# Kyubyong/dc_tts

Hardware: NVIDIA H100
Metric: mel_frames_per_sec (higher is better)
Workload: dtype f32 (decode: fp32 FMA; TextEnc/SSRN: fp16x2 split operands on wgmma, fp32 accumulate)

## Files before the change

### dc_tts_b200/csrc/dctts_api.cu

```cuda
#include "../../include/dctts.h"
#include "kernels.cuh"
#include "kernels_tc.cuh"
#include "kernels_decode.cuh"

#include <cstdio>
#include <cstdlib>
#include <algorithm>
#include <cmath>
#include <cstring>
#include <map>
#include <memory>
#include <stdexcept>
#include <string>
#include <vector>

using namespace dctts;

#define CUDA_CHECK(expr)                                                                     \
    do {                                                                                     \
        cudaError_t _e = (expr);                                                             \
        if (_e != cudaSuccess) {                                                             \
            char _buf[512];                                                                  \
            snprintf(_buf, sizeof(_buf), "%s failed: %s (%s:%d)", #expr, cudaGetErrorString(_e), \
                     __FILE__, __LINE__);                                                    \
// ... 370 lines not shown
    memset(&P, 0, sizeof(P));
    P.nl = (int)nets.size(); P.n_enc = (int)h->audioenc.size();
    std::vector<int> prow = audiodec_rows(h->audiodec, hp.max_T);
    int nch = 0, off = 0;
    for (int li = 0; li < P.nl; ++li) {
        const LayerDev& l = *nets[li];
        DecLayer& L = P.L[li];
        if (l.kind == K_D || !l.causal || (l.cin % 4) || (l.kind == K_HC && (l.cin != d || l.cout != d)) || l.cout % DEC_NC ||
            (li != 0 && l.cin % 128)) { D.why = "persistent decode: unsupported block " + l.scope; return; }
        L.kind = l.kind == K_HC ? 1 : 0; L.cin = l.cin; L.cout = l.cout; L.ntaps = l.size; L.rate = l.rate; L.act = l.act;
        L.cs = l.cout / DEC_NC; L.ns = L.kind ? 2 * L.cs : (L.cs <= 8 ? 8 : roundup(L.cs, 4));
        if (L.ns != 8 && L.ns != 16 && L.ns != 32) { D.why = "persistent decode: unsupported slice width"; return; }
        L.prow = li >= P.n_enc ? prow[li - P.n_enc] : 1;
        if (L.prow > 1 && (L.cout != 256 || (L.ns != 32 && L.ns != 16) || L.prow > 85)) { D.why = "persistent decode: unsupported receptive field"; return; }
        L.ldin = l.cin;
        const int cinp = roundup(l.cin, 128);
        if (l.size > 1 && cinp != 256) { D.why = "persistent decode: multi-tap blocks must have 256 input channels"; return; }
        const int K = l.size * cinp;
        L.krows = std::min(K, DEC_SLOT_F / L.ns);
        const int kr8 = L.krows / 8, sg = 32 / L.ns;
        if (K % L.krows || L.krows % 8 || kr8 * L.ns > DEC_REG_F || kr8 % (8 * sg) || (L.prow > 1 && kr8 % 16)) {
            D.why = "persistent decode: chunk geometry"; return;
        }
        if (L.prow > 1 && (L.prow - 1) + (l.size - 1) * l.rate > 96) { D.why = "persistent decode: receptive field too tall"; return; }
        L.ch0 = nch;
        for (int k0 = 0; k0 < K; k0 += L.krows) {
            if (nch >= DEC_MAXCH) { D.why = "persistent decode: too many weight chunks"; return; }
            DecChunk& c = P.C[nch++];
            c.off = off; c.nfl4 = (short)(L.krows * L.ns / 4); c.k0 = (short)k0; c.krows = (short)L.krows; c.layer = (short)li;
            off += L.krows * L.ns;
        }
        L.nch = nch - L.ch0;
        if (li == P.n_enc - 1) P.nch_enc = nch;
        if (L.prow > 1) { if (P.pyr_ch1 == 0) P.pyr_ch0 = L.ch0; P.pyr_ch1 = nch; }
    }
    if (P.L[P.nl - 1].prow != 1 || P.L[P.n_enc].ntaps != 1 || P.nch_enc <= DEC_NSLOT) { D.why = "persistent decode: unexpected AudioDec shape"; return; }
    for (int li = P.n_enc; li < P.nl; ++li)
        if (P.L[li].prow > 1 && li > P.n_enc && P.L[li - 1].prow <= 1) { D.why = "persistent decode: receptive-field blocks not contiguous"; return; }
    P.nch = nch;
    for (int li = 0; li < P.nl; ++li) {
        const DecLayer& L = P.L[li];
        if (L.prow <= 1) continue;
        if (L.krows % 128 || !((L.ns == 32 && L.ntaps == 3) || (L.ns == 16 && L.ntaps == 1)) ||
            (li == P.n_enc && (L.cin != 2 * d || d != 256)) || (li > P.n_enc && L.cin != 256)) {
            D.why = "persistent decode: tensor-core pre-pass geometry"; return;
        }
        for (int c = L.ch0; c < L.ch0 + L.nch; ++c) { P.C[c].off16 = off; off += L.krows * L.ns; }
// ... 499 lines not shown
    cudaError_t e = cudaGraphInstantiate(&h->ar_exec, graph, 0);
    cudaGraphDestroy(graph);
    CUDA_CHECK(e);
    CUDA_CHECK(cudaGetLastError());
    h->ar_B = B;
}

bool decode_cluster(H* h, int B, int steps, cudaStream_t s) {
    auto& D = h->dec;
    if (!D.ok || h->opt.decode_mode != 1) return false;
    const dctts_hparams& hp = h->hp;
    IntBufs ib = ints(h);
    DecParams P = D.tab;
    for (int li = 0; li < P.nl; ++li) {
        const bool enc = li < P.n_enc;
        P.out_hist[li] = enc ? h->ae_out[li].as<float>() : h->ad_out[li - P.n_enc].as<float>();
        P.in_hist[li] = li == 0 ? nullptr : (li == P.n_enc ? h->rbuf.as<float>() : P.out_hist[li - 1]);
    }
    P.kv = h->kv.as<float>(); P.ybuf = h->ybuf.as<float>(); P.rbuf = h->rbuf.as<float>(); P.pre_scr = D.scr.as<float>();
    decode_plane_halfs(h, h->ws_B, D.pl.as<__half>(), &P);
    P.p_hist = ib.p_hist; P.p_final = D.pfinal.as<int>(); P.stats = D.stats.as<int>();
    P.prof = nullptr;
    P.force_prepass = h->opt.decode_force_prepass != 0;
    if (h->opt.decode_prof) { D.prof.ensure(16 * sizeof(long long)); CUDA_CHECK(cudaMemsetAsync(D.prof.p, 0, 16 * sizeof(long long), s)); P.prof = D.prof.as<long long>(); }
    P.B = B;
    {
        const int mc = std::max(1, D.max_clusters);
        int G = 1;
        while (G < DEC_GMAX && (B + G - 1) / G > mc) ++G;
        P.G = G;
    }
    P.T = hp.max_T; P.N = hp.max_N; P.d = hp.d; P.n_mels = hp.n_mels;
    P.win_size = hp.attention_win_size; P.steps = steps;
    const int n_clusters = (B + P.G - 1) / P.G;
    cudaError_t e = launch_decode_cluster(P, n_clusters, s);
    if (e != cudaSuccess) {
        cudaGetLastError();
        D.ok = false; D.why = std::string("decode_cluster_kernel launch failed: ") + cudaGetErrorString(e);
        return false;
    }
    h->launches += 1;
    D.last_clusters = n_clusters; D.last_moved_frames = -1;
    return true;
}

void text2mel_generate(H* h, const int* L, int B, int steps, float* Y, int* prev_hist,
                       long long* maxatt, float* align, cudaStream_t s) {
// ... 1327 lines not shown
        *value = *slot;
    });
}

int dctts_decode_stats(dctts_handle h, int32_t* moved_frames, int32_t* moved_utterance_frames, int32_t* clusters) {
    return guarded(h, [&] {
        auto& D = h->dec;
        REQUIRE(D.last_clusters > 0, "dctts_decode_stats: no persistent decode has run on this handle");
        if (D.last_moved_frames < 0) {
            std::vector<int> st(2 * (size_t)D.last_clusters);
            CUDA_CHECK(cudaDeviceSynchronize());
            CUDA_CHECK(cudaMemcpy(st.data(), D.stats.p, st.size() * sizeof(int), cudaMemcpyDeviceToHost));
            D.last_moved_frames = 0; D.last_moved_utt = 0;
            for (int c = 0; c < D.last_clusters; ++c) { D.last_moved_frames += st[2 * c]; D.last_moved_utt += st[2 * c + 1]; }
        }
        if (moved_frames) *moved_frames = D.last_moved_frames;
        if (moved_utterance_frames) *moved_utterance_frames = D.last_moved_utt;
        if (clusters) *clusters = D.last_clusters;
    });
}

int dctts_decode_profile(dctts_handle h, int64_t* cycles, int32_t n) {
    return guarded(h, [&] {
        REQUIRE(cycles && n >= 1 && n <= 16, "dctts_decode_profile: bad arguments");
        REQUIRE(h->dec.prof.p, "dctts_decode_profile: no profiled decode has run (set option decode_prof)");
        CUDA_CHECK(cudaDeviceSynchronize());
        long long v[16];
        CUDA_CHECK(cudaMemcpy(v, h->dec.prof.p, sizeof(v), cudaMemcpyDeviceToHost));
        for (int i = 0; i < n; ++i) cycles[i] = v[i];
    });
}

int dctts_malloc(dctts_handle h, void** ptr, int64_t bytes) {
    return guarded(h, [&] { REQUIRE(ptr && bytes > 0, "dctts_malloc: bad arguments"); CUDA_CHECK(cudaMalloc(ptr, (size_t)bytes)); });
}
int dctts_free(dctts_handle h, void* ptr) { return guarded(h, [&] { CUDA_CHECK(cudaFree(ptr)); }); }
int dctts_memcpy_h2d(dctts_handle h, void* dst, const void* src, int64_t bytes, void* stream) {
    return guarded(h, [&] { CUDA_CHECK(cudaMemcpyAsync(dst, src, (size_t)bytes, cudaMemcpyHostToDevice, S(h, stream))); });
}
int dctts_memcpy_d2h(dctts_handle h, void* dst, const void* src, int64_t bytes, void* stream) {
    return guarded(h, [&] { CUDA_CHECK(cudaMemcpyAsync(dst, src, (size_t)bytes, cudaMemcpyDeviceToHost, S(h, stream))); });
}
int dctts_malloc_host(dctts_handle h, void** ptr, int64_t bytes) {
    return guarded(h, [&] { REQUIRE(ptr && bytes > 0, "dctts_malloc_host: bad arguments"); CUDA_CHECK(cudaMallocHost(ptr, (size_t)bytes)); });
}
int dctts_free_host(dctts_handle h, void* ptr) { return guarded(h, [&] { CUDA_CHECK(cudaFreeHost(ptr)); }); }
int dctts_stream_sync(dctts_handle h, void* stream) { return guarded(h, [&] { CUDA_CHECK(cudaStreamSynchronize(S(h, stream))); }); }

}
```

### dc_tts_b200/csrc/kernels_decode.cu

```cuda
#include "kernels_decode.cuh"
#include "tc_ptx.cuh"

#include <cuda_fp16.h>
#include <atomic>
#include <math.h>

namespace dctts {
using namespace ptx;

namespace {

constexpr int NC = DEC_NC, GMAX = DEC_GMAX, NT = DEC_THREADS, NWARP = NT / 32;
constexpr int XLD = 768;
constexpr int PLD = GMAX * 32 + 16;
constexpr int TC_RA = 96;
constexpr int TC_APLANE = 2 * TC_RA * 16;
constexpr int TC_ASTAGE = 2 * TC_APLANE;
constexpr int TC_NSTG = 3;
static_assert(GMAX * NT >= 1024, "red: LayerNorm parameters of the pre-pass");
static_assert(TC_RA == DEC_PL_PAD, "pl_c1 rows are staged as whole slabs");

struct Smem {
    float ring[DEC_NSLOT][NWARP][DEC_REG_F];
    float red[GMAX][NT];
    float xin[2][GMAX][XLD];
    union {
        float pre[2][NC][PLD];
        unsigned char tca[TC_NSTG][TC_ASTAGE];
    };
    float outv[2][GMAX * 32];
    float prm[2][DEC_PRM_F];
    unsigned long long fullw[DEC_NSLOT][NWARP];
    unsigned long long gbar[2];
    unsigned long long sbar[TC_NSTG], abar[TC_NSTG];
    float stat[GMAX][2][2];
    uint32_t tc_baddr[96];
    int n_moved_frames, n_moved_utt;
    DecParams P;
    int p_cur[GMAX], p_prev[GMAX], p_next[GMAX], moved[GMAX];
    int fmoved[2];
    long long prof[16], prof_last;
};

static_assert(sizeof(Smem) + 128 <= 232448, "decode kernel: shared memory budget (227 KB per CTA)");
static_assert(sizeof(float) * 2 * NC * PLD >= TC_NSTG * TC_ASTAGE, "A stages inside pre");

#define LAP(i) do { if constexpr (PROF) { if (threadIdx.x == 0) { const long long now_ = clock64(); S.prof[i] += now_ - S.prof_last; S.prof_last = now_; } } } while (0)
enum { LP_START = 0, LP_WAIT = 1, LP_GEMV = 2, LP_RELEASE = 3, LP_GATHER = 4, LP_CBAR = 5, LP_LN = 6, LP_MIX = 7, LP_ATT = 8,
       LP_PYR_ATT = 9, LP_PYR_GEMM = 10, LP_PYR_LN = 11, LP_PYR_BAR = 12, LP_FRAME = 13 };

__device__ __forceinline__ float warp_sum(float v) {
#pragma unroll
    for (int o = 16; o > 0; o >>= 1) v += __shfl_xor_sync(0xffffffffu, v, o);
    return v;
}
__device__ __forceinline__ float sigmoid_acc(float x) { return 1.0f / (1.0f + expf(-x)); }
__device__ __forceinline__ float sigmoid_fast(float x) { return __fdividef(1.0f, 1.0f + __expf(-x)); }

__device__ __forceinline__ void cp_async16(void* dst, const void* src, bool valid) {
    const int sz = valid ? 16 : 0;
    asm volatile("cp.async.cg.shared.global [%0], [%1], 16, %2;" :: "r"(smem_u32(dst)), "l"(src), "r"(sz) : "memory");
}
__device__ __forceinline__ void cp_async_commit() { asm volatile("cp.async.commit_group;" ::: "memory"); }
template <int N> __device__ __forceinline__ void cp_async_wait() { asm volatile("cp.async.wait_group %0;" :: "n"(N) : "memory"); }

__device__ __forceinline__ void bulk_g2s(void* dst, const void* src, uint32_t bytes, unsigned long long* bar) {
    asm volatile("cp.async.bulk.shared::cluster.global.mbarrier::complete_tx::bytes [%0], [%1], %2, [%3];"
                 :: "r"(smem_u32(dst)), "l"(src), "r"(bytes), "r"(smem_u32(bar)) : "memory");
}
__device__ __forceinline__ void bulk_s2peer(uint32_t dst_cluster, const void* src, uint32_t bytes, uint32_t bar_cluster) {
    asm volatile("cp.async.bulk.shared::cluster.shared::cta.mbarrier::complete_tx::bytes [%0], [%1], %2, [%3];"
                 :: "r"(dst_cluster), "r"(smem_u32(src)), "r"(bytes), "r"(bar_cluster) : "memory");
}
__device__ __forceinline__ void cluster_sync_all() { cluster_arrive(); cluster_wait(); }
__device__ __forceinline__ void fence_proxy_async_global() { asm volatile("fence.proxy.async.global;" ::: "memory"); }

__device__ __forceinline__ size_t pl_idx(int nslab, int rows, int b, int c, int t) {
    return ((size_t)(b * nslab + (c >> 4)) * 4 + ((c >> 3) & 1)) * (size_t)rows * 8 + (size_t)(t + DEC_PL_PAD) * 8 + (c & 7);
}
__device__ __forceinline__ void split_h(float v, __half& hi, __half& lo) {
    hi = __float2half_rn(v);
    lo = __float2half_rn(v - __half2float(hi));
}
__device__ __forceinline__ void store_split8(__half* p, const float (&v)[8]) {
    __align__(16) __half hi[8];
    __align__(16) __half lo[8];
#pragma unroll
    for (int i = 0; i < 8; ++i) split_h(v[i], hi[i], lo[i]);
    *reinterpret_cast<uint4*>(p) = *reinterpret_cast<const uint4*>(hi);
    *reinterpret_cast<uint4*>(p + TC_APLANE / 2) = *reinterpret_cast<const uint4*>(lo);
}
// ... 339 lines not shown
    r.n = j - r.t_lo;
    r.total = r.n * __popc(r.mask);
    return r;
}
__device__ __forceinline__ void pre_row_of(const PreRows& r, int m, int& g, int& t) {
    const int k = m / r.n;
    unsigned mk = r.mask;
    for (int i = 0; i < k; ++i) mk &= mk - 1;
    g = __ffs(mk) - 1;
    t = r.t_lo + (m - k * r.n);
}
__device__ __forceinline__ int pre_off_of(const PreRows& r, int g) { return r.n * __popc(r.mask & ((1u << g) - 1u)); }

__device__ __forceinline__ void pyr_tc_table(const DecParams& P, Smem& S, int li, unsigned pos0) {
    const DecLayer& l = P.L[li];
    const int nslab = l.cin / 16, spc = l.krows / 16, spr = spc / 8, slab_f = 16 * l.ns;
    const int sid = (int)threadIdx.x;
    if (sid < l.ntaps * nslab) {
        const int c = sid / spc, wi = sid - c * spc, reg = wi / spr, jj = wi - reg * spr;
        S.tc_baddr[sid] = (smem_u32(&S.ring[(pos0 + c) % DEC_NSLOT][reg][jj * slab_f]) & 0x3FFFFu) >> 4;
    }
}

template <int NS, int NTAPS, int MH>
__device__ __forceinline__ void pyr_mma_rows(const DecParams& P, Smem& S, int li, unsigned& use, int& stg, int n_out, int rank,
                                             float* scr_rows) {
    const DecLayer& l = P.L[li];
    const int nslab = l.cin / 16, lane = threadIdx.x & 31, w4 = (threadIdx.x >> 5) & 3;
    const bool leader = (threadIdx.x & 127) == 0;
    unsigned char* As = &S.tca[0][0];
    const uint64_t dA0 = gmma_desc_noswz(0, TC_RA * 16, 128), dB0 = gmma_desc_noswz(0, (uint32_t)NS * 16, 128);
    const uint32_t a_base = (smem_u32(As) & 0x3FFFFu) >> 4, b_lo = (uint32_t)NS * 2, tap_step = (uint32_t)l.rate;
    float acc[MH][NS / 2];
#pragma unroll
    for (int m = 0; m < MH; ++m)
#pragma unroll
        for (int i = 0; i < NS / 2; ++i) acc[m][i] = 0.f;
    int prev = 0;
#pragma unroll 1
    for (int ks = 0; ks < nslab; ++ks) {
        uint32_t bt[NTAPS];
#pragma unroll
        for (int tap = 0; tap < NTAPS; ++tap) bt[tap] = S.tc_baddr[tap * nslab + ks];
        const uint32_t aa = a_base + (uint32_t)stg * (TC_ASTAGE >> 4);
        mbar_wait(bar64(&S.abar[stg]), use & 1u);
        wg_fence();
#pragma unroll
        for (int tap = 0; tap < NTAPS; ++tap) {
            const uint64_t db_hi = dB0 | bt[tap], db_lo = dB0 | (bt[tap] + b_lo);
#pragma unroll
            for (int m = 0; m < MH; ++m) {
                const uint32_t a = aa + (uint32_t)tap * tap_step + 64u * m;
                const uint64_t da_hi = dA0 | a, da_lo = dA0 | (a + (TC_APLANE >> 4));
                wgmma_f16<NS / 16>(acc[m], da_hi, db_hi, (ks | tap) != 0);
                wgmma_f16<NS / 16>(acc[m], da_hi, db_lo, 1u);
                wgmma_f16<NS / 16>(acc[m], da_lo, db_hi, 1u);
            }
        }
        wg_commit();
        wg_wait<1>();
        if (ks > 0 && leader) mbar_arrive(bar64(&S.sbar[prev]));
        prev = stg;
        if (++stg == TC_NSTG) { stg = 0; ++use; }
    }
    wg_wait<0>();
#pragma unroll
    for (int m = 0; m < MH; ++m) wg_fence_regs(acc[m]);
    if (leader) mbar_arrive(bar64(&S.sbar[prev]));
    const float inv = P.inv_scale[li];
    const float* bs = P.bias[li];
#pragma unroll
    for (int m = 0; m < MH; ++m)
#pragma unroll
        for (int h = 0; h < 2; ++h) {
            const int row = 64 * m + 16 * w4 + (lane >> 2) + 8 * h;
            if (row >= n_out) continue;
            float* orow = scr_rows + (size_t)row * 512;
#pragma unroll
            for (int i = 0; i < NS / 8; ++i) {
                const int n = i * 8 + 2 * (lane & 3), hf = n >> 4, nn = n & 15;
                const int col = hf * 256 + rank * 16 + nn, bi = hf * l.cout + rank * 16 + nn;
                const float2 bq = __ldg(reinterpret_cast<const float2*>(bs + bi));
                *reinterpret_cast<float2*>(orow + col) = make_float2(fmaf(acc[m][i * 4 + 2 * h], inv, bq.x),
                                                                     fmaf(acc[m][i * 4 + 2 * h + 1], inv, bq.y));
            }
        }
}

__device__ __forceinline__ void pyr_tc_utt(const DecParams& P, Smem& S, int li, unsigned q0, int b, int t_lo, int n_out,
                                        int rank, float* scr_rows, const __half* c1) {
    const DecLayer& l = P.L[li];
    const int tid = threadIdx.x, warp = tid >> 5;
    unsigned use = q0 / TC_NSTG;
    int stg = (int)(q0 - use * TC_NSTG);
    if (tid == 0) {
        const int halo = (l.ntaps - 1) * l.rate, n_src = n_out + halo;
        const int nslab = l.cin / 16;
        const size_t run = (size_t)P.pl_rows * 8;
        const __half* src = c1 ? c1 : P.pl_hist[li] + pl_idx(nslab, P.pl_rows, b, 0, t_lo - halo);
        const size_t sstep = c1 ? (size_t)TC_ASTAGE / 2 : 4 * run;
        const uint32_t rb = (uint32_t)n_src * 16;
        fence_proxy_async_global();
#pragma unroll 1
        for (int ks = 0; ks < nslab; ++ks, src += sstep) {
            if (use > 0) mbar_wait(bar64(&S.sbar[stg]), (use - 1) & 1u);
            unsigned char* dst = &S.tca[stg][0];
            if (c1) {
                mbar_expect_tx(bar64(&S.abar[stg]), TC_ASTAGE);
                bulk_g2s(dst, src, TC_ASTAGE, &S.abar[stg]);
            } else {
                mbar_expect_tx(bar64(&S.abar[stg]), 4 * rb);
#pragma unroll
                for (int r = 0; r < 4; ++r)
                    bulk_g2s(dst + (r >> 1) * TC_APLANE + (r & 1) * (TC_RA * 16), src + r * run, rb, &S.abar[stg]);
            }
            if (++stg == TC_NSTG) { stg = 0; ++use; }
        }
    } else if (warp >= 4) {
        if (l.ns == 32) {
            if (n_out > 64) pyr_mma_rows<32, 3, 2>(P, S, li, use, stg, n_out, rank, scr_rows);
            else pyr_mma_rows<32, 3, 1>(P, S, li, use, stg, n_out, rank, scr_rows);
        } else {
            if (n_out > 64) pyr_mma_rows<16, 1, 2>(P, S, li, use, stg, n_out, rank, scr_rows);
            else pyr_mma_rows<16, 1, 1>(P, S, li, use, stg, n_out, rank, scr_rows);
        }
    }
}

__device__ __forceinline__ void pyr_ln(const DecParams& P, Smem& S, int li, int b0, const PreRows& rl, int rank, const float* scr) {
    const DecLayer& l = P.L[li];
    const int warp = threadIdx.x >> 5, lane = threadIdx.x & 31;
    const float* prm = &S.red[0][0];
    const float fC = 256.f;
    for (int m = rank * NWARP + warp; m < rl.total; m += NC * NWARP) {
        int g, t; pre_row_of(rl, m, g, t);
        const float* y = scr + (size_t)m * 512;
        const size_t row = (size_t)(b0 + g) * P.T + t;
        float z[2][8];
#pragma unroll
        for (int hf = 0; hf < 2; ++hf) {
            if (hf > l.kind) break;
            const float4 a = ldcg4(y + hf * 256 + lane * 4), b = ldcg4(y + hf * 256 + 128 + lane * 4);
            float v[8] = {a.x, a.y, a.z, a.w, b.x, b.y, b.z, b.w};
            float s = 0.f;
#pragma unroll
            for (int i = 0; i < 8; ++i) s += v[i];
            const float mean = warp_sum(s) / fC;
            float qd = 0.f;
// ... 43 lines not shown
                float qv[8], ctx[8];
                const float4 q0 = ldcg4(Qh + row * P.d + lane * 8), q1 = ldcg4(Qh + row * P.d + lane * 8 + 4);
                qv[0] = q0.x; qv[1] = q0.y; qv[2] = q0.z; qv[3] = q0.w; qv[4] = q1.x; qv[5] = q1.y; qv[6] = q1.z; qv[7] = q1.w;
                attend_row(P, qv, b0 + g, S.p_cur[g], lane, ctx);
                float* rr = P.rbuf + row * (2 * P.d);
                *reinterpret_cast<float4*>(rr + lane * 8) = make_float4(ctx[0], ctx[1], ctx[2], ctx[3]);
                *reinterpret_cast<float4*>(rr + lane * 8 + 4) = make_float4(ctx[4], ctx[5], ctx[6], ctx[7]);
                *reinterpret_cast<float4*>(rr + P.d + lane * 8) = q0;
                *reinterpret_cast<float4*>(rr + P.d + lane * 8 + 4) = q1;
                __half* cs = c1s + (size_t)g * c1_utt + (size_t)(lane >> 1) * (TC_ASTAGE / 2) + (lane & 1) * (TC_RA * 8) + (t - ra.t_lo) * 8;
                store_split8(cs, ctx);
                store_split8(cs + (size_t)(P.d >> 4) * (TC_ASTAGE / 2), qv);
            }
            fence_proxy_async_global();
            cluster_sync_all();
            LAP(LP_PYR_ATT);
            for (int lp = P.n_enc; lp < P.nl && P.L[lp].prow > 1; ++lp) {
                const DecLayer& l = P.L[lp];
                for (int c = 0; c < l.nch; ++c) {
                    const unsigned pp = st.pos + c;
                    if (lane < NWARP) mbar_wait(bar64(&S.fullw[pp % DEC_NSLOT][lane]), (pp / DEC_NSLOT) & 1u);
                }
                __syncwarp();
                const PreRows rl = pre_rows(S, G, j, l.prow);
                if (rl.n > 0) {
                    pyr_tc_table(P, S, lp, st.pos);
                    __syncthreads();
                    for (int g = 0; g < G; ++g) {
                        if (!((rl.mask >> g) & 1u)) continue;
                        float* rows = scr + (size_t)pre_off_of(rl, g) * 512;
                        pyr_tc_utt(P, S, lp, st.tcq, b0 + g, rl.t_lo, rl.n, rank, rows, lp == P.n_enc ? c1s + (size_t)g * c1_utt : nullptr);
                        st.tcq += l.cin / 16;
                    }
                }
                __syncthreads();
                for (int c = 0; c < l.nch; ++c) {
                    if (lane == 0) { fence_proxy_async_smem(); stream_issue(P, S, st, st.prod, (int)(st.pos % DEC_NSLOT), warp); }
                    stream_advance(P, S, st);
                }
                for (int i = tid; i < 256; i += NT)
                    *reinterpret_cast<float4*>(&S.red[0][0] + i * 4) = __ldg(reinterpret_cast<const float4*>(P.lnp[lp]) + i);
                LAP(LP_PYR_GEMM);
                cluster_sync_all();
                LAP(LP_PYR_BAR);
                pyr_ln(P, S, lp, b0, rl, rank, scr);
                LAP(LP_PYR_LN);
                fence_proxy_async_global();
                cluster_sync_all();
                LAP(LP_PYR_BAR);
            }
            return st;
}

template <bool PROF, int GT>
__global__ void __cluster_dims__(DEC_NC, 1, 1) __launch_bounds__(DEC_THREADS, 1)
decode_cluster_kernel(const __grid_constant__ DecParams Pc) {
    extern __shared__ __align__(128) unsigned char smem_raw[];
    Smem& S = *reinterpret_cast<Smem*>(smem_raw);
    const int tid = threadIdx.x, warp = tid >> 5, lane = tid & 31;
    {
        const int* src = reinterpret_cast<const int*>(&Pc);
        int* dst = reinterpret_cast<int*>(&S.P);
        for (int i = tid; i < (int)(sizeof(DecParams) / 4); i += NT) dst[i] = src[i];
    }
    __syncthreads();
    const DecParams& P = S.P;
    const int rank = (int)cluster_ctarank();
    const int cluster = blockIdx.x / NC;
    const int b0 = cluster * P.G;
    const int G = min(P.G, P.B - b0);
    float* scr = P.pre_scr + (size_t)cluster * P.G * 85 * 512;
    __half* c1s = P.pl_c1 + (size_t)cluster * P.G * (P.L[P.n_enc].cin / 16) * (TC_ASTAGE / 2);

    if (tid == 0) {
        for (int s = 0; s < DEC_NSLOT; ++s)
            for (int w = 0; w < NWARP; ++w) mbar_init(bar64(&S.fullw[s][w]), 1);
        mbar_init(bar64(&S.gbar[0]), 1); mbar_init(bar64(&S.gbar[1]), 1);
        for (int i = 0; i < TC_NSTG; ++i) { mbar_init(bar64(&S.sbar[i]), 1); mbar_init(bar64(&S.abar[i]), 1); }
        fence_mbar_init();
    }
    for (int i = tid; i < 2 * GMAX * XLD; i += NT) (&S.xin[0][0][0])[i] = 0.f;
    for (int i = tid; i < 2 * NC * PLD; i += NT) (&S.pre[0][0][0])[i] = 0.f;
    if (tid < GMAX) { S.p_cur[tid] = 0; S.p_prev[tid] = 0; S.p_next[tid] = 0; S.moved[tid] = 0; }
    if (tid < 2) S.fmoved[tid] = 0;
    if (tid < 16) S.prof[tid] = 0;
    if (tid == 0) { S.n_moved_frames = 0; S.n_moved_utt = 0; }
    __syncthreads();

    Stream st;
    st.base = P.wstream + (size_t)rank * P.stream_len;
    st.prod = Cur{0, 0, 0}; st.pos = 0; st.tcq = 0;
    for (int s = 0; s < DEC_NSLOT; ++s) {
        if (lane == 0) stream_issue(P, S, st, st.prod, s, warp);
        cur_next(P, S, st.prod);
    }
    prefetch_params(P, S, 0, rank);
    cp_async_commit();
    cluster_sync_all();

    int cb = 0;
    unsigned lcount = 0;
    __syncthreads();
    if (tid == 0) S.prof_last = clock64();
    for (int j = 0; j < P.steps; ++j) {
        if (tid < GMAX) S.moved[tid] = (tid < G && j > 0 && (P.force_prepass || S.p_cur[tid] != S.p_prev[tid])) ? 1 : 0;
        if (tid == 0) {
            int any = 0;
            for (int g = 0; g < G; ++g) any |= (j > 0 && (P.force_prepass || S.p_cur[g] != S.p_prev[g])) ? 1 : 0;
// ... 12 lines not shown
#pragma unroll
            for (int i = 0; i < 8; ++i) qv[i] = S.xin[cb][g][lane * 8 + i];
            const int amax = attend_row(P, qv, b0 + g, S.p_cur[g], lane, ctx);
            if (lane == 0) S.p_next[g] = amax;
#pragma unroll
            for (int i = 0; i < 8; ++i) { S.xin[cb ^ 1][g][lane * 8 + i] = ctx[i]; S.xin[cb ^ 1][g][P.d + lane * 8 + i] = qv[i]; }
        }
        cb ^= 1;
        LAP(LP_ATT);

        if (any_moved) st = prepass<PROF>(P, S, st, j, b0, G, rank, scr, c1s);
        }
        cb = layer_row<PROF, GT>(P, S, st, li, j, b0, G, rank, cb, lcount);
        }

        __syncthreads();
        if (tid < GMAX) { S.p_prev[tid] = S.p_cur[tid]; S.p_cur[tid] = S.p_next[tid]; }
        fence_proxy_async_global();
        cluster_sync_all();
        LAP(LP_FRAME);
    }
    if (rank == 0 && tid < G) P.p_final[b0 + tid] = S.p_cur[tid];
    if (rank == 0 && tid == 0 && P.stats) { P.stats[2 * cluster] = S.n_moved_frames; P.stats[2 * cluster + 1] = S.n_moved_utt; }
    if (PROF && P.prof && cluster == 0 && rank == 0 && tid < 16) P.prof[tid] = S.prof[tid];
    cp_async_wait<0>();
    cluster_sync_all();
}

size_t decode_smem_bytes() { return sizeof(Smem) + 128; }

using DecKernel = void (*)(DecParams);
static DecKernel decode_kernel_of(bool prof, int G) {
    switch (G) {
        case 1: return prof ? decode_cluster_kernel<true, 1> : decode_cluster_kernel<false, 1>;
        case 2: return prof ? decode_cluster_kernel<true, 2> : decode_cluster_kernel<false, 2>;
        case 3: return prof ? decode_cluster_kernel<true, 3> : decode_cluster_kernel<false, 3>;
        case 4: return prof ? decode_cluster_kernel<true, 4> : decode_cluster_kernel<false, 4>;
        default: return prof ? decode_cluster_kernel<true, 5> : decode_cluster_kernel<false, 5>;
    }
}
static_assert(DEC_GMAX == 5, "decode_kernel_of: one instantiation per utterance count");

static cudaError_t decode_prepare() {
    static std::atomic<bool> done[64];
    int dev = 0;
    cudaError_t e = cudaGetDevice(&dev);
    if (e != cudaSuccess) return e;
// ... 37 lines not shown
```

### dc_tts_b200/csrc/kernels_decode.cuh

```cuda
#pragma once
#include <cuda_fp16.h>
#include <cuda_runtime.h>
#include <stdint.h>

namespace dctts {

constexpr int DEC_NC = 16;
constexpr int DEC_GMAX = 5;
constexpr int DEC_THREADS = 256;
constexpr int DEC_NSLOT = 3;
constexpr int DEC_REG_F = 1536;
constexpr int DEC_SLOT_F = 8 * DEC_REG_F;
constexpr int DEC_MAXL = 24;
constexpr int DEC_MAXCH = 48;
constexpr int DEC_PRM_F = 1024 + 64;
constexpr int DEC_PL_PAD = 96;

struct DecLayer {
    int kind;
    int cin;
    int cout;
    int ntaps, rate;
    int act;
    int ns;
    int cs;
    int ch0, nch;
    int krows;
    int prow;
    int ldin;
};
struct DecChunk { int off; int off16; short nfl4; short k0; short krows; short layer; };

struct DecParams {
    DecLayer L[DEC_MAXL];
    DecChunk C[DEC_MAXCH];
    const float* in_hist[DEC_MAXL];
    float* out_hist[DEC_MAXL];
    const float* lnp[DEC_MAXL];
    const float* bias[DEC_MAXL];
// ... 25 lines not shown
```

### dc_tts_b200/csrc/tc_ptx.cuh

```cuda
#pragma once
#include <cuda_runtime.h>
#include <stdint.h>

namespace dctts { namespace ptx {

__device__ __forceinline__ uint32_t smem_u32(const void* p) {
    return static_cast<uint32_t>(__cvta_generic_to_shared(p));
}
__device__ __forceinline__ bool elect_one() {
    uint32_t pred = 0;
    asm volatile("{\n\t.reg .pred P;\n\telect.sync _|P, 0xffffffff;\n\tselp.u32 %0, 1, 0, P;\n\t}" : "=r"(pred));
    return pred != 0;
}

__device__ __forceinline__ void mbar_init(uint64_t* bar, uint32_t count) {
    asm volatile("mbarrier.init.shared::cta.b64 [%0], %1;" :: "r"(smem_u32(bar)), "r"(count));
}
__device__ __forceinline__ void fence_mbar_init() { asm volatile("fence.mbarrier_init.release.cluster;" ::: "memory"); }
__device__ __forceinline__ void mbar_expect_tx(uint64_t* bar, uint32_t bytes) {
    asm volatile("mbarrier.arrive.expect_tx.shared::cta.b64 _, [%0], %1;" :: "r"(smem_u32(bar)), "r"(bytes) : "memory");
}
__device__ __forceinline__ bool mbar_try_wait(uint64_t* bar, uint32_t parity) {
    uint32_t ok;
    asm volatile(
// ... 117 lines not shown
    static_assert(SW == 128 || SW == 64, "swizzle span");
    uint64_t d = 0;
    d |= static_cast<uint64_t>((smem_addr & 0x3FFFF) >> 4);
    d |= 1ull << 16;
    d |= static_cast<uint64_t>((8 * SW) >> 4) << 32;
    d |= static_cast<uint64_t>(SW == 128 ? 1 : 2) << 62;
    return d;
}
__device__ __forceinline__ uint64_t gmma_desc_noswz(uint32_t smem_addr, uint32_t lbo_bytes, uint32_t sbo_bytes) {
    uint64_t d = 0;
    d |= static_cast<uint64_t>((smem_addr & 0x3FFFF) >> 4);
    d |= static_cast<uint64_t>(lbo_bytes >> 4) << 16;
    d |= static_cast<uint64_t>(sbo_bytes >> 4) << 32;
    return d;
}

__device__ __forceinline__ void mbar_arrive(uint64_t* bar) {
    asm volatile("mbarrier.arrive.shared::cta.b64 _, [%0];" :: "r"(smem_u32(bar)) : "memory");
}
__device__ __forceinline__ uint32_t mapa(uint32_t smem_addr, uint32_t rank);
__device__ __forceinline__ void mbar_arrive_cluster(uint64_t* bar, uint32_t rank) {
    asm volatile("mbarrier.arrive.release.cluster.shared::cluster.b64 _, [%0];" :: "r"(mapa(smem_u32(bar), rank)) : "memory");
}
__device__ __forceinline__ void named_sync(int id, int n) { asm volatile("bar.sync %0, %1;" :: "r"(id), "r"(n) : "memory"); }

__device__ __forceinline__ uint32_t cluster_ctarank() { uint32_t r; asm volatile("mov.u32 %0, %%cluster_ctarank;" : "=r"(r)); return r; }
__device__ __forceinline__ uint32_t cluster_nctarank() { uint32_t r; asm volatile("mov.u32 %0, %%cluster_nctarank;" : "=r"(r)); return r; }
__device__ __forceinline__ void cluster_arrive() { asm volatile("barrier.cluster.arrive.release.aligned;" ::: "memory"); }
__device__ __forceinline__ void cluster_wait() { asm volatile("barrier.cluster.wait.acquire.aligned;" ::: "memory"); }
__device__ __forceinline__ uint32_t mapa(uint32_t smem_addr, uint32_t rank) {
    uint32_t r;
    asm volatile("mapa.shared::cluster.u32 %0, %1, %2;" : "=r"(r) : "r"(smem_addr), "r"(rank));
    return r;
}
__device__ __forceinline__ float4 ld_cluster_f4(uint32_t addr) {
    float4 v;
    asm volatile("ld.shared::cluster.v4.f32 {%0, %1, %2, %3}, [%4];" : "=f"(v.x), "=f"(v.y), "=f"(v.z), "=f"(v.w) : "r"(addr) : "memory");
    return v;
}
__device__ __forceinline__ void st_cluster_f4(uint32_t addr, float a, float b, float c, float d) {
    asm volatile("st.shared::cluster.v4.f32 [%0], {%1, %2, %3, %4};" :: "r"(addr), "f"(a), "f"(b), "f"(c), "f"(d) : "memory");
}

}}
```

### dc_tts_b200/engine.py

```python
import ctypes as C

import numpy as np
import torch

from . import _lib
from .hyperparams import Hyperparams as hp
from .params import check_params


class DcttsError(RuntimeError):
    pass


def _ptr(t):
    return C.c_void_p(0) if t is None else C.c_void_p(t.data_ptr())


class Engine:
    def __init__(self, device=0, hparams=hp):
        self._lib = _lib.load()
        if not torch.cuda.is_available():
            raise DcttsError("dc_tts_b200 needs a CUDA device (sm_90a); there is no CPU fallback")
        self.device = torch.device("cuda", device)
        self.hp = hparams
# ... 61 lines not shown
    def restore(self, text2mel_dir, ssrn_dir=None):
        from .checkpoint import Saver, latest_checkpoint
        Saver(var_list=["Text2Mel"]).restore(self, latest_checkpoint(text2mel_dir))
        Saver(var_list=["SSRN", "gs"]).restore(self, latest_checkpoint(ssrn_dir if ssrn_dir is not None else text2mel_dir))
        return self.commit_params()

    def set_tensor_path(self, mode):
        self._check(self._lib.dctts_set_tensor_path(self._h, int(mode)), "dctts_set_tensor_path")

    def set_option(self, name, value):
        self._check(self._lib.dctts_set_option(self._h, name.encode(), int(value)), "dctts_set_option(%s)" % name)

    def get_option(self, name):
        v = C.c_int32(0)
        self._check(self._lib.dctts_get_option(self._h, name.encode(), C.byref(v)), "dctts_get_option(%s)" % name)
        return int(v.value)

    def decode_stats(self):
        a, b, c = C.c_int32(0), C.c_int32(0), C.c_int32(0)
        self._check(self._lib.dctts_decode_stats(self._h, C.byref(a), C.byref(b), C.byref(c)), "dctts_decode_stats")
        return int(a.value), int(b.value), int(c.value)

    def decode_profile(self):
        v = (C.c_int64 * 14)()
        self._check(self._lib.dctts_decode_profile(self._h, v, 14), "dctts_decode_profile")
        names = ["start", "stream_wait", "gemv", "release", "gather", "cluster_barrier", "layernorm", "mix", "attention",
                 "re_attention", "re_gemm", "re_layernorm", "re_barriers", "frame"]
        return dict(zip(names, [int(x) for x in v]))

    def reserve(self, batch):
        self._check(self._lib.dctts_reserve(self._h, int(batch)), "dctts_reserve")

    def bench_block(self, scope, B, L, iters=5, warmup=2):
        ms = (C.c_float * 8)()
        n = C.c_int32(0)
        self._check(self._lib.dctts_bench_block(self._h, scope.encode(), B, L, iters, warmup, ms, C.byref(n),
                                                self._stream()), "dctts_bench_block")
        return [float(ms[i]) for i in range(n.value)]

    def conv_gemm(self, impl, mode, X, K, Wd, N, shifts, out, bias=None, accumulate=0):
        ts = [X, Wd, out] + ([bias] if bias is not None else [])
        if not all(t.is_cuda and t.dtype == torch.float32 and t.stride(-1) == 1 for t in ts):
            raise DcttsError("conv_gemm: CUDA float32 tensors with a unit inner stride expected")
        B, L = X.shape[0], X.shape[1]
        rows_ok = X.stride(0) == L * X.stride(1) and (mode == 1 or out.stride(0) == L * out.stride(1))
        taps_ok = (Wd.stride(0) == K * Wd.stride(1)) if mode == 0 else (out.stride(0) == K * out.stride(1))
        dy_ok = mode == 0 or (Wd.shape[0] == B and Wd.shape[1] == L and Wd.stride(0) == L * Wd.stride(1))
        if not (rows_ok and taps_ok and dy_ok):
            raise DcttsError("conv_gemm: rows or taps of a tensor are not evenly pitched")
        sh = (C.c_int32 * len(shifts))(*[int(s) for s in shifts])
# ... 385 lines not shown
```

Measured before the change: 129,300.

## Multicast pyramid A-tile loads across cluster and pack utterances per stage

The pyramid re-encode path now issues the A-operand bulk copies from only one CTA per stage, round-robin across the cluster, using cluster multicast. Each consumer CTA releases the stage by arriving remotely on the issuing CTA's barrier. The stage count goes from 3 to 6 and the row pad from 96 to 88. A packed path loads all utterances' three tap images into one stage, so a single wgmma pass covers the whole group instead of one pass per utterance. Finer profiling buckets are also added. The goal is less redundant global-to-shared traffic and fewer serial per-utterance MMA passes, at the cost of more complex cross-CTA barrier accounting and more shared memory.

```diff
diff --git a/dc_tts_b200/csrc/dctts_api.cu b/dc_tts_b200/csrc/dctts_api.cu
--- a/dc_tts_b200/csrc/dctts_api.cu
+++ b/dc_tts_b200/csrc/dctts_api.cu
@@ -416,7 +416,7 @@
         if (K % L.krows || L.krows % 8 || kr8 * L.ns > DEC_REG_F || kr8 % (8 * sg) || (L.prow > 1 && kr8 % 16)) {
             D.why = "persistent decode: chunk geometry"; return;
         }
-        if (L.prow > 1 && (L.prow - 1) + (l.size - 1) * l.rate > 96) { D.why = "persistent decode: receptive field too tall"; return; }
+        if (L.prow > 1 && (L.prow - 1) + (l.size - 1) * l.rate > DEC_PL_PAD) { D.why = "persistent decode: receptive field too tall"; return; }
         L.ch0 = nch;
         for (int k0 = 0; k0 < K; k0 += L.krows) {
             if (nch >= DEC_MAXCH) { D.why = "persistent decode: too many weight chunks"; return; }
@@ -962,7 +962,7 @@
     P.p_hist = ib.p_hist; P.p_final = D.pfinal.as<int>(); P.stats = D.stats.as<int>();
     P.prof = nullptr;
     P.force_prepass = h->opt.decode_force_prepass != 0;
-    if (h->opt.decode_prof) { D.prof.ensure(16 * sizeof(long long)); CUDA_CHECK(cudaMemsetAsync(D.prof.p, 0, 16 * sizeof(long long), s)); P.prof = D.prof.as<long long>(); }
+    if (h->opt.decode_prof) { D.prof.ensure(DEC_NPROF * sizeof(long long)); CUDA_CHECK(cudaMemsetAsync(D.prof.p, 0, DEC_NPROF * sizeof(long long), s)); P.prof = D.prof.as<long long>(); }
     P.B = B;
     {
         const int mc = std::max(1, D.max_clusters);
@@ -2336,10 +2336,10 @@
 
 int dctts_decode_profile(dctts_handle h, int64_t* cycles, int32_t n) {
     return guarded(h, [&] {
-        REQUIRE(cycles && n >= 1 && n <= 16, "dctts_decode_profile: bad arguments");
+        REQUIRE(cycles && n >= 1 && n <= DEC_NPROF, "dctts_decode_profile: bad arguments");
         REQUIRE(h->dec.prof.p, "dctts_decode_profile: no profiled decode has run (set option decode_prof)");
         CUDA_CHECK(cudaDeviceSynchronize());
-        long long v[16];
+        long long v[DEC_NPROF];
         CUDA_CHECK(cudaMemcpy(v, h->dec.prof.p, sizeof(v), cudaMemcpyDeviceToHost));
         for (int i = 0; i < n; ++i) cycles[i] = v[i];
     });
diff --git a/dc_tts_b200/csrc/kernels_decode.cu b/dc_tts_b200/csrc/kernels_decode.cu
--- a/dc_tts_b200/csrc/kernels_decode.cu
+++ b/dc_tts_b200/csrc/kernels_decode.cu
@@ -3,6 +3,7 @@
 
 #include <cuda_fp16.h>
 #include <atomic>
+#include <cstddef>
 #include <math.h>
 
 namespace dctts {
@@ -13,10 +14,15 @@
 constexpr int NC = DEC_NC, GMAX = DEC_GMAX, NT = DEC_THREADS, NWARP = NT / 32;
 constexpr int XLD = 768;
 constexpr int PLD = GMAX * 32 + 16;
-constexpr int TC_RA = 96;
+constexpr int TC_RA = DEC_PL_PAD;
 constexpr int TC_APLANE = 2 * TC_RA * 16;
 constexpr int TC_ASTAGE = 2 * TC_APLANE;
-constexpr int TC_NSTG = 3;
+constexpr int TC_NSTG = 6;
+constexpr int gcd_c(int a, int b) { return b == 0 ? a : gcd_c(b, a % b); }
+constexpr unsigned TC_QCYC = NC / gcd_c(NC, TC_NSTG) * TC_NSTG;
+constexpr int TC_PR = 24;
+constexpr int TC_PTAP = 2 * 2 * TC_PR * 16;
+static_assert(3 * TC_PTAP <= TC_ASTAGE, "packed tap images inside a stage");
 static_assert(GMAX * NT >= 1024, "red: LayerNorm parameters of the pre-pass");
 static_assert(TC_RA == DEC_PL_PAD, "pl_c1 rows are staged as whole slabs");
 
@@ -39,15 +45,18 @@
     DecParams P;
     int p_cur[GMAX], p_prev[GMAX], p_next[GMAX], moved[GMAX];
     int fmoved[2];
-    long long prof[16], prof_last;
+    long long prof[DEC_NPROF], prof_last;
 };
 
 static_assert(sizeof(Smem) + 128 <= 232448, "decode kernel: shared memory budget (227 KB per CTA)");
-static_assert(sizeof(float) * 2 * NC * PLD >= TC_NSTG * TC_ASTAGE, "A stages inside pre");
+static_assert(offsetof(Smem, tca) + sizeof(Smem::tca) + 128 * 16 <= sizeof(Smem), "A tile reads past the stages");
 
 #define LAP(i) do { if constexpr (PROF) { if (threadIdx.x == 0) { const long long now_ = clock64(); S.prof[i] += now_ - S.prof_last; S.prof_last = now_; } } } while (0)
 enum { LP_START = 0, LP_WAIT = 1, LP_GEMV = 2, LP_RELEASE = 3, LP_GATHER = 4, LP_CBAR = 5, LP_LN = 6, LP_MIX = 7, LP_ATT = 8,
-       LP_PYR_ATT = 9, LP_PYR_GEMM = 10, LP_PYR_LN = 11, LP_PYR_BAR = 12, LP_FRAME = 13 };
+       LP_PYR_ATT = 9, LP_PYR_WTS = 10, LP_PYR_TABLE = 11, LP_PYR_STAGE = 12, LP_PYR_DRAIN = 13, LP_PYR_REFILL = 14,
+       LP_PYR_LN = 15, LP_PYR_BAR = 16, LP_FRAME = 17,
+       LP_WG_AWAIT = 18, LP_WG_MMA = 19, LP_WG_EPI = 20, LP_COUNT };
+static_assert(LP_COUNT <= DEC_NPROF, "lap buckets");
 
 __device__ __forceinline__ float warp_sum(float v) {
 #pragma unroll
@@ -67,6 +76,10 @@
 __device__ __forceinline__ void bulk_g2s(void* dst, const void* src, uint32_t bytes, unsigned long long* bar) {
     asm volatile("cp.async.bulk.shared::cluster.global.mbarrier::complete_tx::bytes [%0], [%1], %2, [%3];"
                  :: "r"(smem_u32(dst)), "l"(src), "r"(bytes), "r"(smem_u32(bar)) : "memory");
+}
+__device__ __forceinline__ void bulk_g2s_mc(void* dst, const void* src, uint32_t bytes, unsigned long long* bar, uint16_t mask) {
+    asm volatile("cp.async.bulk.shared::cluster.global.mbarrier::complete_tx::bytes.multicast::cluster [%0], [%1], %2, [%3], %4;"
+                 :: "r"(smem_u32(dst)), "l"(src), "r"(bytes), "r"(smem_u32(bar)), "h"(mask) : "memory");
 }
 __device__ __forceinline__ void bulk_s2peer(uint32_t dst_cluster, const void* src, uint32_t bytes, uint32_t bar_cluster) {
     asm volatile("cp.async.bulk.shared::cluster.shared::cta.mbarrier::complete_tx::bytes [%0], [%1], %2, [%3];"
@@ -452,28 +465,38 @@
     }
 }
 
-template <int NS, int NTAPS, int MH>
-__device__ __forceinline__ void pyr_mma_rows(const DecParams& P, Smem& S, int li, unsigned& use, int& stg, int n_out, int rank,
+template <bool PROF, int NS, int NTAPS, int MH, bool PACKED>
+__device__ __forceinline__ void pyr_mma_rows(const DecParams& P, Smem& S, int li, unsigned q0, int n_out, int rank,
                                              float* scr_rows) {
     const DecLayer& l = P.L[li];
     const int nslab = l.cin / 16, lane = threadIdx.x & 31, w4 = (threadIdx.x >> 5) & 3;
     const bool leader = (threadIdx.x & 127) == 0;
+    long long t_prof = 0;
+    auto wlap = [&](int i) {
+        if constexpr (PROF) { if (leader) { const long long now = clock64(); if (i >= 0) S.prof[i] += now - t_prof; t_prof = now; } }
+    };
+    wlap(-1);
     unsigned char* As = &S.tca[0][0];
-    const uint64_t dA0 = gmma_desc_noswz(0, TC_RA * 16, 128), dB0 = gmma_desc_noswz(0, (uint32_t)NS * 16, 128);
-    const uint32_t a_base = (smem_u32(As) & 0x3FFFFu) >> 4, b_lo = (uint32_t)NS * 2, tap_step = (uint32_t)l.rate;
+    const uint64_t dA0 = gmma_desc_noswz(0, (PACKED ? TC_PR : TC_RA) * 16, 128), dB0 = gmma_desc_noswz(0, (uint32_t)NS * 16, 128);
+    const uint32_t a_base = (smem_u32(As) & 0x3FFFFu) >> 4, b_lo = (uint32_t)NS * 2;
+    const uint32_t tap_step = PACKED ? (uint32_t)(TC_PTAP >> 4) : (uint32_t)l.rate;
+    constexpr uint32_t a_lo = (PACKED ? 2 * TC_PR * 16 : TC_APLANE) >> 4;
     float acc[MH][NS / 2];
 #pragma unroll
     for (int m = 0; m < MH; ++m)
 #pragma unroll
         for (int i = 0; i < NS / 2; ++i) acc[m][i] = 0.f;
-    int prev = 0;
+    auto release = [&](unsigned q) { mbar_arrive_remote(bar64(&S.sbar[q % TC_NSTG]), (q + TC_NSTG) % NC); };
+    unsigned q = q0;
 #pragma unroll 1
-    for (int ks = 0; ks < nslab; ++ks) {
+    for (int ks = 0; ks < nslab; ++ks, ++q) {
         uint32_t bt[NTAPS];
 #pragma unroll
         for (int tap = 0; tap < NTAPS; ++tap) bt[tap] = S.tc_baddr[tap * nslab + ks];
-        const uint32_t aa = a_base + (uint32_t)stg * (TC_ASTAGE >> 4);
-        mbar_wait(bar64(&S.abar[stg]), use & 1u);
+        const unsigned stg = q % TC_NSTG;
+        const uint32_t aa = a_base + stg * (TC_ASTAGE >> 4);
+        mbar_wait(bar64(&S.abar[stg]), (q / TC_NSTG) & 1u);
+        wlap(LP_WG_AWAIT);
         wg_fence();
 #pragma unroll
         for (int tap = 0; tap < NTAPS; ++tap) {
@@ -481,7 +504,7 @@
 #pragma unroll
             for (int m = 0; m < MH; ++m) {
                 const uint32_t a = aa + (uint32_t)tap * tap_step + 64u * m;
-                const uint64_t da_hi = dA0 | a, da_lo = dA0 | (a + (TC_APLANE >> 4));
+                const uint64_t da_hi = dA0 | a, da_lo = dA0 | (a + a_lo);
                 wgmma_f16<NS / 16>(acc[m], da_hi, db_hi, (ks | tap) != 0);
                 wgmma_f16<NS / 16>(acc[m], da_hi, db_lo, 1u);
                 wgmma_f16<NS / 16>(acc[m], da_lo, db_hi, 1u);
@@ -489,14 +512,14 @@
         }
         wg_commit();
         wg_wait<1>();
-        if (ks > 0 && leader) mbar_arrive(bar64(&S.sbar[prev]));
-        prev = stg;
-        if (++stg == TC_NSTG) { stg = 0; ++use; }
+        if (ks > 0 && leader) release(q - 1);
+        wlap(LP_WG_MMA);
     }
     wg_wait<0>();
 #pragma unroll
     for (int m = 0; m < MH; ++m) wg_fence_regs(acc[m]);
-    if (leader) mbar_arrive(bar64(&S.sbar[prev]));
+    if (leader) release(q - 1);
+    wlap(LP_WG_MMA);
     const float inv = P.inv_scale[li];
     const float* bs = P.bias[li];
 #pragma unroll
@@ -515,14 +538,14 @@
                                                                      fmaf(acc[m][i * 4 + 2 * h + 1], inv, bq.y));
             }
         }
-}
-
+    wlap(LP_WG_EPI);
+}
+
+template <bool PROF>
 __device__ __forceinline__ void pyr_tc_utt(const DecParams& P, Smem& S, int li, unsigned q0, int b, int t_lo, int n_out,
                                         int rank, float* scr_rows, const __half* c1) {
     const DecLayer& l = P.L[li];
     const int tid = threadIdx.x, warp = tid >> 5;
-    unsigned use = q0 / TC_NSTG;
-    int stg = (int)(q0 - use * TC_NSTG);
     if (tid == 0) {
         const int halo = (l.ntaps - 1) * l.rate, n_src = n_out + halo;
         const int nslab = l.cin / 16;
@@ -530,30 +553,71 @@
         const __half* src = c1 ? c1 : P.pl_hist[li] + pl_idx(nslab, P.pl_rows, b, 0, t_lo - halo);
         const size_t sstep = c1 ? (size_t)TC_ASTAGE / 2 : 4 * run;
         const uint32_t rb = (uint32_t)n_src * 16;
+        const uint16_t all = (uint16_t)((1u << NC) - 1u);
         fence_proxy_async_global();
+        unsigned q = q0;
 #pragma unroll 1
-        for (int ks = 0; ks < nslab; ++ks, src += sstep) {
-            if (use > 0) mbar_wait(bar64(&S.sbar[stg]), (use - 1) & 1u);
+        for (int ks = 0; ks < nslab; ++ks, src += sstep, ++q) {
+            const unsigned stg = q % TC_NSTG, use = q / TC_NSTG;
+            if (use > 0) mbar_wait(bar64(&S.abar[stg]), (use - 1) & 1u);
+            mbar_expect_tx(bar64(&S.abar[stg]), c1 ? (uint32_t)TC_ASTAGE : 4 * rb);
+            if (q % NC != (unsigned)rank) continue;
+            if (use > 0) mbar_wait(bar64(&S.sbar[stg]), ((q - TC_NSTG) / TC_QCYC) & 1u);
             unsigned char* dst = &S.tca[stg][0];
             if (c1) {
-                mbar_expect_tx(bar64(&S.abar[stg]), TC_ASTAGE);
-                bulk_g2s(dst, src, TC_ASTAGE, &S.abar[stg]);
+                bulk_g2s_mc(dst, src, TC_ASTAGE, &S.abar[stg], all);
             } else {
-                mbar_expect_tx(bar64(&S.abar[stg]), 4 * rb);
 #pragma unroll
                 for (int r = 0; r < 4; ++r)
-                    bulk_g2s(dst + (r >> 1) * TC_APLANE + (r & 1) * (TC_RA * 16), src + r * run, rb, &S.abar[stg]);
-            }
-            if (++stg == TC_NSTG) { stg = 0; ++use; }
+                    bulk_g2s_mc(dst + (r >> 1) * TC_APLANE + (r & 1) * (TC_RA * 16), src + r * run, rb, &S.abar[stg], all);
+            }
         }
     } else if (warp >= 4) {
         if (l.ns == 32) {
-            if (n_out > 64) pyr_mma_rows<32, 3, 2>(P, S, li, use, stg, n_out, rank, scr_rows);
-            else pyr_mma_rows<32, 3, 1>(P, S, li, use, stg, n_out, rank, scr_rows);
+            if (n_out > 64) pyr_mma_rows<PROF, 32, 3, 2, false>(P, S, li, q0, n_out, rank, scr_rows);
+            else pyr_mma_rows<PROF, 32, 3, 1, false>(P, S, li, q0, n_out, rank, scr_rows);
         } else {
-            if (n_out > 64) pyr_mma_rows<16, 1, 2>(P, S, li, use, stg, n_out, rank, scr_rows);
-            else pyr_mma_rows<16, 1, 1>(P, S, li, use, stg, n_out, rank, scr_rows);
-        }
+            if (n_out > 64) pyr_mma_rows<PROF, 16, 1, 2, false>(P, S, li, q0, n_out, rank, scr_rows);
+            else pyr_mma_rows<PROF, 16, 1, 1, false>(P, S, li, q0, n_out, rank, scr_rows);
+        }
+    }
+}
+
+template <bool PROF>
+__device__ __forceinline__ void pyr_tc_packed(const DecParams& P, Smem& S, int li, unsigned q0, int b0, const PreRows& rl,
+                                           int rank, float* scr) {
+    const DecLayer& l = P.L[li];
+    const int tid = threadIdx.x, warp = tid >> 5;
+    if (tid == 0) {
+        const int halo = (l.ntaps - 1) * l.rate, nslab = l.cin / 16, nu = __popc(rl.mask);
+        const size_t run = (size_t)P.pl_rows * 8;
+        const uint32_t rb = (uint32_t)rl.n * 16;
+        const uint16_t all = (uint16_t)((1u << NC) - 1u);
+        fence_proxy_async_global();
+        unsigned q = q0;
+#pragma unroll 1
+        for (int ks = 0; ks < nslab; ++ks, ++q) {
+            const unsigned stg = q % TC_NSTG, use = q / TC_NSTG;
+            if (use > 0) mbar_wait(bar64(&S.abar[stg]), (use - 1) & 1u);
+            mbar_expect_tx(bar64(&S.abar[stg]), (uint32_t)(3 * 4 * nu) * rb);
+            if (q % NC != (unsigned)rank) continue;
+            if (use > 0) mbar_wait(bar64(&S.sbar[stg]), ((q - TC_NSTG) / TC_QCYC) & 1u);
+            unsigned char* dst = &S.tca[stg][0];
+            unsigned mk = rl.mask;
+#pragma unroll 1
+            for (int k = 0; k < nu; ++k, mk &= mk - 1) {
+                const int g = __ffs(mk) - 1;
+                const __half* src = P.pl_hist[li] + pl_idx(nslab, P.pl_rows, b0 + g, ks * 16, rl.t_lo - halo);
+#pragma unroll 1
+                for (int tap = 0; tap < 3; ++tap)
+#pragma unroll
+                    for (int r = 0; r < 4; ++r)
+                        bulk_g2s_mc(dst + tap * TC_PTAP + r * (TC_PR * 16) + k * rb, src + (size_t)tap * l.rate * 8 + r * run, rb,
+                                    &S.abar[stg], all);
+            }
+        }
+    } else if (warp >= 4) {
+        pyr_mma_rows<PROF, 32, 3, 1, true>(P, S, li, q0, rl.total, rank, scr);
     }
 }
 
@@ -643,25 +707,32 @@
                     if (lane < NWARP) mbar_wait(bar64(&S.fullw[pp % DEC_NSLOT][lane]), (pp / DEC_NSLOT) & 1u);
                 }
                 __syncwarp();
+                LAP(LP_PYR_WTS);
                 const PreRows rl = pre_rows(S, G, j, l.prow);
                 if (rl.n > 0) {
                     pyr_tc_table(P, S, lp, st.pos);
                     __syncthreads();
-                    for (int g = 0; g < G; ++g) {
+                    LAP(LP_PYR_TABLE);
+                    if (l.ns == 32 && (l.prow - 1) * GMAX <= TC_PR) {
+                        pyr_tc_packed<PROF>(P, S, lp, st.tcq, b0, rl, rank, scr);
+                        st.tcq += l.cin / 16;
+                    } else for (int g = 0; g < G; ++g) {
                         if (!((rl.mask >> g) & 1u)) continue;
                         float* rows = scr + (size_t)pre_off_of(rl, g) * 512;
-                        pyr_tc_utt(P, S, lp, st.tcq, b0 + g, rl.t_lo, rl.n, rank, rows, lp == P.n_enc ? c1s + (size_t)g * c1_utt : nullptr);
+                        pyr_tc_utt<PROF>(P, S, lp, st.tcq, b0 + g, rl.t_lo, rl.n, rank, rows, lp == P.n_enc ? c1s + (size_t)g * c1_utt : nullptr);
                         st.tcq += l.cin / 16;
                     }
+                    LAP(LP_PYR_STAGE);
                 }
                 __syncthreads();
+                LAP(LP_PYR_DRAIN);
                 for (int c = 0; c < l.nch; ++c) {
                     if (lane == 0) { fence_proxy_async_smem(); stream_issue(P, S, st, st.prod, (int)(st.pos % DEC_NSLOT), warp); }
                     stream_advance(P, S, st);
                 }
                 for (int i = tid; i < 256; i += NT)
                     *reinterpret_cast<float4*>(&S.red[0][0] + i * 4) = __ldg(reinterpret_cast<const float4*>(P.lnp[lp]) + i);
-                LAP(LP_PYR_GEMM);
+                LAP(LP_PYR_REFILL);
                 cluster_sync_all();
                 LAP(LP_PYR_BAR);
                 pyr_ln(P, S, lp, b0, rl, rank, scr);
@@ -697,14 +768,14 @@
         for (int s = 0; s < DEC_NSLOT; ++s)
             for (int w = 0; w < NWARP; ++w) mbar_init(bar64(&S.fullw[s][w]), 1);
         mbar_init(bar64(&S.gbar[0]), 1); mbar_init(bar64(&S.gbar[1]), 1);
-        for (int i = 0; i < TC_NSTG; ++i) { mbar_init(bar64(&S.sbar[i]), 1); mbar_init(bar64(&S.abar[i]), 1); }
+        for (int i = 0; i < TC_NSTG; ++i) { mbar_init(bar64(&S.sbar[i]), NC); mbar_init(bar64(&S.abar[i]), 1); }
         fence_mbar_init();
     }
     for (int i = tid; i < 2 * GMAX * XLD; i += NT) (&S.xin[0][0][0])[i] = 0.f;
     for (int i = tid; i < 2 * NC * PLD; i += NT) (&S.pre[0][0][0])[i] = 0.f;
     if (tid < GMAX) { S.p_cur[tid] = 0; S.p_prev[tid] = 0; S.p_next[tid] = 0; S.moved[tid] = 0; }
     if (tid < 2) S.fmoved[tid] = 0;
-    if (tid < 16) S.prof[tid] = 0;
+    if (tid < DEC_NPROF) S.prof[tid] = 0;
     if (tid == 0) { S.n_moved_frames = 0; S.n_moved_utt = 0; }
     __syncthreads();
 
@@ -763,7 +834,7 @@
     }
     if (rank == 0 && tid < G) P.p_final[b0 + tid] = S.p_cur[tid];
     if (rank == 0 && tid == 0 && P.stats) { P.stats[2 * cluster] = S.n_moved_frames; P.stats[2 * cluster + 1] = S.n_moved_utt; }
-    if (PROF && P.prof && cluster == 0 && rank == 0 && tid < 16) P.prof[tid] = S.prof[tid];
+    if (PROF && P.prof && cluster == 0 && rank == 0 && tid < DEC_NPROF) P.prof[tid] = S.prof[tid];
     cp_async_wait<0>();
     cluster_sync_all();
 }
diff --git a/dc_tts_b200/csrc/kernels_decode.cuh b/dc_tts_b200/csrc/kernels_decode.cuh
--- a/dc_tts_b200/csrc/kernels_decode.cuh
+++ b/dc_tts_b200/csrc/kernels_decode.cuh
@@ -14,7 +14,8 @@
 constexpr int DEC_MAXL = 24;
 constexpr int DEC_MAXCH = 48;
 constexpr int DEC_PRM_F = 1024 + 64;
-constexpr int DEC_PL_PAD = 96;
+constexpr int DEC_PL_PAD = 88;
+constexpr int DEC_NPROF = 24;
 
 struct DecLayer {
     int kind;
diff --git a/dc_tts_b200/csrc/tc_ptx.cuh b/dc_tts_b200/csrc/tc_ptx.cuh
--- a/dc_tts_b200/csrc/tc_ptx.cuh
+++ b/dc_tts_b200/csrc/tc_ptx.cuh
@@ -163,6 +163,9 @@
 __device__ __forceinline__ void mbar_arrive_cluster(uint64_t* bar, uint32_t rank) {
     asm volatile("mbarrier.arrive.release.cluster.shared::cluster.b64 _, [%0];" :: "r"(mapa(smem_u32(bar), rank)) : "memory");
 }
+__device__ __forceinline__ void mbar_arrive_remote(uint64_t* bar, uint32_t rank) {
+    asm volatile("mbarrier.arrive.shared::cluster.b64 _, [%0];" :: "r"(mapa(smem_u32(bar), rank)) : "memory");
+}
 __device__ __forceinline__ void named_sync(int id, int n) { asm volatile("bar.sync %0, %1;" :: "r"(id), "r"(n) : "memory"); }
 
 __device__ __forceinline__ uint32_t cluster_ctarank() { uint32_t r; asm volatile("mov.u32 %0, %%cluster_ctarank;" : "=r"(r)); return r; }
diff --git a/dc_tts_b200/engine.py b/dc_tts_b200/engine.py
--- a/dc_tts_b200/engine.py
+++ b/dc_tts_b200/engine.py
@@ -107,10 +107,11 @@
         return int(a.value), int(b.value), int(c.value)
 
     def decode_profile(self):
-        v = (C.c_int64 * 14)()
-        self._check(self._lib.dctts_decode_profile(self._h, v, 14), "dctts_decode_profile")
         names = ["start", "stream_wait", "gemv", "release", "gather", "cluster_barrier", "layernorm", "mix", "attention",
-                 "re_attention", "re_gemm", "re_layernorm", "re_barriers", "frame"]
+                 "re_attention", "re_weights", "re_table", "re_stage", "re_drain", "re_refill", "re_layernorm", "re_barriers",
+                 "frame", "wg_a_wait", "wg_mma", "wg_epilogue"]
+        v = (C.c_int64 * len(names))()
+        self._check(self._lib.dctts_decode_profile(self._h, v, len(names)), "dctts_decode_profile")
         return dict(zip(names, [int(x) for x in v]))
 
     def reserve(self, batch):
```

New measurement: 136,700 (median of 6 runs). 1.06x the previous value.
